# lucagiorgetti/Laplace-DQN-Snake-game

Measured on NVIDIA B200. Metric: snake_env_steps_per_sec, higher is better.
Workload: dtype u64 bitboards -> f32 obs

## Files before the change

laplace-dqn-snake-game_b200/csrc/snake_env.cu:

```cuda
#include <stdarg.h>
#include <string.h>

#include <new>
#include <mutex>
#include <type_traits>
#include <unordered_map>

#include <cuda.h>

#include "common.h"

#ifndef SNK_OBS_STORE_MODE
#define SNK_OBS_STORE_MODE 1
#endif
#if SNK_OBS_STORE_MODE == 1
#define SNK_OBS_STORE(p, v) (*(p) = (v))
#elif SNK_OBS_STORE_MODE == 2
#define SNK_OBS_STORE(p, v) __stwt((p), (v))
#else
#define SNK_OBS_STORE(p, v) __stcs((p), (v))
#endif

namespace snk {

static thread_local char g_err[512];
char *err_buf() { return g_err; }
int fail(int code, const char *fmt, ...) {
    va_list ap;
    va_start(ap, fmt);
    vsnprintf(g_err, sizeof(g_err), fmt, ap);
    va_end(ap);
    return code;
}

#ifndef SNK_TPB
#define SNK_TPB 256
#endif
#ifndef SNK_MINB
#define SNK_MINB 1
#endif
#ifndef SNK_UNROLL
#define SNK_UNROLL 4
#endif
constexpr int PHASE_B_UNROLL = SNK_UNROLL;
constexpr int TPB = SNK_TPB;
constexpr int MAX_FOOD = 64;
constexpr int PLANE_WORDS = 16;

constexpr int M_HR = 0, M_HC = 4, M_TR = 8, M_TC = 12, M_FR = 16, M_FC = 20, M_PFR = 24, M_PFC = 28;
constexpr int M_PD = 32, M_LEN = 34, M_T = 41, M_DONE = 51, M_ERR = 52;

constexpr u64 wall_bits(int lo_hi) {
    u64 lo = 0, hi = 0;
    for (int c = 0; c < 10; c++)
        for (int r = 0; r < 10; r++)
            if (r == 0 || r == 9 || c == 0 || c == 9) {
                int k = r + 10 * c;
                if (k < 64) lo |= 1ull << k; else hi |= 1ull << (k - 64);
            }
    return lo_hi ? hi : lo;
}
constexpr u64 WALL_LO = wall_bits(0), WALL_HI = wall_bits(1);

constexpr u64 INIT_OCC = (1ull << (6 + 0)) | (1ull << (7 + 0));
constexpr u64 INIT_MISC = (7ull << M_HR) | (1ull << M_HC) | (8ull << M_TR) | (1ull << M_TC) | (3ull << M_FR) |
                          (4ull << M_FC) | (3ull << M_PFR) | (4ull << M_PFC) | (0ull << M_PD) | (2ull << M_LEN);

struct FoodTable {
    uint8_t bit[MAX_FOOD];
    int n;
    __host__ __device__ u64 mask() const { return n >= 64 ? ~0ull : ((1ull << n) - 1ull); }
};

struct EnvState {
    u64 *occ, *pocc, *clo, *chi, *cons, *misc;
    float *ret;
};

__host__ __device__ constexpr int obs_bytes(int fmt) {
    switch (fmt) {
        case SNK_OBS_F32: return 800;
        case SNK_OBS_I8: return 200;
        case SNK_OBS_I64: return 1600;
        case SNK_OBS_PACKED2: return 50;
        case SNK_OBS_BITS: return 24;
        default: return 0;
    }
}

struct StepOutputs {
    float *reward;
    uint8_t *done;
    void *obs;
    uint8_t *mask;
    float *ep_return;
    int32_t *ep_score;
};

struct StepArgs {
    EnvState s;
    const uint8_t *act;
    const float *q;
    const float *u;
    const uint8_t *ridx;
    float eps;
    uint8_t *act_out;
    StepOutputs out;
    long long env_begin, env_end;
    u64 seed, step_counter;
    int auto_reset, is_abs;
    uint4 *sink;
    long long sink_base, sink_cap, sink_n;
    FoodTable food;
};

constexpr int REC_U4 = 8;

__host__ __device__ __forceinline__ u64 splitmix64(u64 x) {
    x += 0x9E3779B97F4A7C15ull;
    x = (x ^ (x >> 30)) * 0xBF58476D1CE4E5B9ull;
    x = (x ^ (x >> 27)) * 0x94D049BB133111EBull;
    return x ^ (x >> 31);
}

__device__ __forceinline__ void dir_delta(int d, int &dr, int &dc) {
    int s = (d & 1) ? 1 : -1;
    dr = (d & 2) ? 0 : s;
    dc = (d & 2) ? s : 0;
// ... 21 lines not shown
    if (b != b) return true;
    if (a < b) return true;
    if (a == b) return (__float_as_uint(a) >> 31) && !(__float_as_uint(b) >> 31);
    return false;
}
__device__ __forceinline__ int select_idx(float q0, float q1, float q2, float eps, float u, int ridx) {
    if (u < eps) return ridx;
    int best = 0;
    float qb = q0;
    if (jl_isless(qb, q1)) { best = 1; qb = q1; }
    if (jl_isless(qb, q2)) { best = 2; }
    return best;
}
__device__ __forceinline__ void internal_draw(u64 seed, u64 step, long long env, float &u, int &ridx) {
    u64 x = splitmix64(seed ^ splitmix64((u64)env * 0x100000001B3ull + step));
    u = (float)(x >> 40) * 5.9604644775390625e-08f;
    ridx = (int)((x & 0xFFFFFFull) % 3ull);
}

__device__ __forceinline__ void to_full(u64 occ, u64 &lo, u64 &hi) {
    u64 b0 = occ & 0xFF, b1 = (occ >> 8) & 0xFF, b2 = (occ >> 16) & 0xFF, b3 = (occ >> 24) & 0xFF;
    u64 b4 = (occ >> 32) & 0xFF, b5 = (occ >> 40) & 0xFF, b6 = (occ >> 48) & 0xFF, b7 = occ >> 56;
    lo = (b0 << 11) | (b1 << 21) | (b2 << 31) | (b3 << 41) | (b4 << 51) | (b5 << 61);
    hi = (b5 >> 3) | (b6 << 7) | (b7 << 17);
}
__device__ __forceinline__ void set_k(int r, int c, u64 &lo, u64 &hi) {
    int k = r + 10 * c;
    u64 b = 1ull << (k & 63);
    if (k < 64) lo |= b; else hi |= b;
}
__device__ __forceinline__ void board_bits(u64 occ, int fr, int fc, bool has_head, int hr, int hc, u64 &p0lo, u64 &p0hi,
                                           u64 &p1lo, u64 &p1hi) {
    u64 slo, shi;
    to_full(occ, slo, shi);
    if (has_head) set_k(hr, hc, slo, shi);
    u64 flo = WALL_LO, fhi = WALL_HI;
    if (fr != 0) set_k(fr, fc, flo, fhi);
    p0lo = slo | WALL_LO; p0hi = shi | WALL_HI;
    p1lo = flo & ~slo; p1hi = fhi & ~shi;
}
__device__ __forceinline__ u64 spread_nibbles(uint32_t x) {
    u64 v = x;
    v = (v | (v << 16)) & 0x0000FFFF0000FFFFull;
    v = (v | (v << 8)) & 0x00FF00FF00FF00FFull;
    v = (v | (v << 4)) & 0x0F0F0F0F0F0F0F0Full;
    return v;
}
__device__ __forceinline__ u64 unit_bytes(uint32_t p0, uint32_t p1) {
    const uint32_t ev = (p0 & 0x0F0F0F0Fu) | ((p1 << 4) & 0xF0F0F0F0u);
    const uint32_t od = ((p0 >> 4) & 0x0F0F0F0Fu) | (p1 & 0xF0F0F0F0u);
    return (u64)__byte_perm(ev, od, 0x5140) | ((u64)__byte_perm(ev, od, 0x7362) << 32);
}
template <bool PERM>
__device__ __forceinline__ u64 unit_word(uint32_t p0, uint32_t p1) {
    return PERM ? unit_bytes(p0, p1) : (spread_nibbles(p0) | (spread_nibbles(p1) << 4));
}
template <bool PERM = true>
__device__ __forceinline__ void board_planes(u64 occ, int fr, int fc, bool has_head, int hr, int hc, uint32_t *dst) {
    u64 p0lo, p0hi, p1lo, p1hi;
    board_bits(occ, fr, fc, has_head, hr, hc, p0lo, p0hi, p1lo, p1hi);
    u64 *d = reinterpret_cast<u64 *>(dst);
    d[0] = unit_word<PERM>((uint32_t)p0lo, (uint32_t)p1lo);
    d[1] = unit_word<PERM>((uint32_t)(p0lo >> 32), (uint32_t)(p1lo >> 32));
    d[2] = unit_word<PERM>((uint32_t)p0hi, (uint32_t)p1hi);
    d[3] = unit_word<PERM>((uint32_t)(p0hi >> 32), (uint32_t)(p1hi >> 32));
}
__device__ __forceinline__ void board_planes_reg(u64 occ, int fr, int fc, bool has_head, int hr, int hc, uint4 &a, uint4 &b) {
    u64 p0lo, p0hi, p1lo, p1hi;
    board_bits(occ, fr, fc, has_head, hr, hc, p0lo, p0hi, p1lo, p1hi);
    a = make_uint4((uint32_t)p0lo, (uint32_t)(p0lo >> 32), (uint32_t)p0hi, (uint32_t)(p0hi >> 32));
    b = make_uint4((uint32_t)p1lo, (uint32_t)(p1lo >> 32), (uint32_t)p1hi, (uint32_t)(p1hi >> 32));
}

__device__ __forceinline__ int cell_code(const uint32_t *pl, int k) {
    const uint32_t b = reinterpret_cast<const uint8_t *>(pl)[k >> 2];
    const int j = k & 3;
    return (int)(((b >> j) & 1u) | (((b >> (4 + j)) & 1u) << 1));
}
__device__ __forceinline__ int code_value(int code) { return code == 3 ? -1 : code; }

struct ObsTables {
    float4 f32[256];
};
template <int OBS>
__device__ __forceinline__ void fill_tables(ObsTables &tb, int tid, int nt = TPB) {
    if (OBS == SNK_OBS_F32 || OBS == SNK_OBS_I8 || OBS == SNK_OBS_PACKED2) {
        for (int i = tid; i < 256; i += nt) {
            int n0 = i & 15, n1 = i >> 4;
            float v[4];
            uint32_t bytes = 0, packed = 0;
            for (int j = 0; j < 4; j++) {
                int code = ((n0 >> j) & 1) | (((n1 >> j) & 1) << 1);
                v[j] = (float)code_value(code);
                bytes |= (uint32_t)(uint8_t)(int8_t)code_value(code) << (8 * j);
                packed |= (uint32_t)code << (2 * j);
            }
            if (OBS == SNK_OBS_F32) tb.f32[i] = make_float4(v[0], v[1], v[2], v[3]);
            else if (OBS == SNK_OBS_I8) reinterpret_cast<uint32_t *>(tb.f32)[i] = bytes;
            else reinterpret_cast<uint8_t *>(tb.f32)[i] = (uint8_t)packed;
        }
    }
}

template <bool STREAM, typename T>
__device__ __forceinline__ void obs_store(T *p, const T &v) {
    if (STREAM) __stcs(p, v); else SNK_OBS_STORE(p, v);
}
__device__ __forceinline__ uint32_t unit_index(const uint32_t *s_planes, int j) {
    const int e = (int)(((unsigned)j * 5243u) >> 18);
    const int qq = j - e * 50;
    const int f = qq >= 25;
    return reinterpret_cast<const uint8_t *>(s_planes)[e * (PLANE_WORDS * 4) + f * 32 + (qq - 25 * f)];
}
template <int OBS, int NT = TPB, int UNROLL = PHASE_B_UNROLL, bool STREAM = false>
__device__ __forceinline__ void expand_obs(void *obs, long long env0, int n_local, const uint32_t *s_planes,
                                           const ObsTables &tb, int tid) {
    if (OBS == SNK_OBS_F32) {
        const int total = n_local * 50;
        float4 *o32 = reinterpret_cast<float4 *>(obs) + env0 * 50;
#pragma unroll UNROLL
        for (int j = tid; j < total; j += NT) obs_store<STREAM>(o32 + j, tb.f32[unit_index(s_planes, j)]);
    } else if (OBS == SNK_OBS_I8) {
        constexpr int GP = NT / 25;
        uint8_t *base = reinterpret_cast<uint8_t *>(obs) + env0 * 200;
        const int n_pairs = (NT % 25 > 10) ? 0 : n_local >> 1;
        if ((reinterpret_cast<uintptr_t>(base) & 15u) == 0) {
            if (tid < GP * 25) {
                const int p0 = tid / 25, w = tid - 25 * p0;
                int off[4];
#pragma unroll
                for (int k = 0; k < 4; k++) {
                    const int uu = 4 * w + k, e2 = uu >= 50, qq = uu - 50 * e2;
                    off[k] = e2 * (PLANE_WORDS * 4) + (qq >= 25 ? 7 : 0) + qq;
                }
                const uint8_t *src = reinterpret_cast<const uint8_t *>(s_planes) + p0 * (2 * PLANE_WORDS * 4);
                const uint32_t *t32 = reinterpret_cast<const uint32_t *>(tb.f32);
                uint4 *o = reinterpret_cast<uint4 *>(base);
#pragma unroll 2
                for (int p = p0; p < n_pairs; p += GP, src += GP * (2 * PLANE_WORDS * 4))
                    obs_store<STREAM>(o + p * 25 + w, make_uint4(t32[src[off[0]]], t32[src[off[1]]], t32[src[off[2]]], t32[src[off[3]]]));
            }
        }
        const int done_units = (reinterpret_cast<uintptr_t>(base) & 15u) == 0 ? n_pairs * 100 : 0;
        for (int j = done_units + tid; j < n_local * 50; j += NT)
            reinterpret_cast<uint32_t *>(base)[j] = reinterpret_cast<const uint32_t *>(tb.f32)[unit_index(s_planes, j)];
    } else if (OBS == SNK_OBS_PACKED2) {
        uint8_t *base = reinterpret_cast<uint8_t *>(obs) + env0 * 50;
        const int total = n_local * 50;
        int done_units = 0;
        if ((reinterpret_cast<uintptr_t>(base) & 15u) == 0) {
            const int nvec = total / 16;
            uint4 *o = reinterpret_cast<uint4 *>(base);
#pragma unroll 2
            for (int v = tid; v < nvec; v += NT) {
                uint32_t w[4];
#pragma unroll
                for (int k = 0; k < 4; k++) {
                    uint32_t x = 0;
#pragma unroll
                    for (int b = 0; b < 4; b++)
                        x |= (uint32_t)reinterpret_cast<const uint8_t *>(tb.f32)[unit_index(s_planes, v * 16 + k * 4 + b)] << (8 * b);
                    w[k] = x;
                }
                obs_store<STREAM>(o + v, make_uint4(w[0], w[1], w[2], w[3]));
            }
            done_units = nvec * 16;
        }
        for (int j = done_units + tid; j < total; j += NT) base[j] = reinterpret_cast<const uint8_t *>(tb.f32)[unit_index(s_planes, j)];
    } else if (OBS == SNK_OBS_I64) {
        const int total = n_local * 100;
        longlong2 *o = reinterpret_cast<longlong2 *>(obs) + env0 * 100;
        for (int j = tid; j < total; j += NT) {
            int e = j / 100;
            int p = j - e * 100;
            int f = p >= 50;
            int k = 2 * (p - 50 * f);
            const uint32_t *pl = s_planes + e * PLANE_WORDS + f * 8;
            longlong2 v;
            v.x = code_value(cell_code(pl, k));
            v.y = code_value(cell_code(pl, k + 1));
            obs_store<STREAM>(o + j, v);
        }
    }
}

__device__ __forceinline__ uint32_t losing_mask3(u64 occ, u64 cons, int hr, int hc, int tr, int tc, int fr, int fc,
                                                 int pd, int t, u64 list_mask, const uint8_t *s_food_bit, int &err) {
    const bool cap = t >= 499;
    const u64 occ_nt = occ & ~(1ull << ((tr - 1) + 8 * (tc - 1)));
    uint32_t m = 0;
#pragma unroll
    for (int k = 0; k < 3; k++) {
        int d = av_dir(pd, k), dr, dc;
        dir_delta(d, dr, dc);
        int nr = hr + dr, nc = hc + dc;
        bool lose;
        if (nr == 0 || nr == 9 || nc == 0 || nc == 9) {
            lose = true;
        } else {
            int b = (nr - 1) + 8 * (nc - 1);
            if (fr != 0 && nr == fr && nc == fc) {
                lose = cap;
                if (food_search(occ | (1ull << b), cons, list_mask, s_food_bit) == -1) err |= SNK_ENV_ERR_FOOD;
            } else {
// ... 41 lines not shown
}
__device__ __forceinline__ void env_store(const Env &e, const EnvState &s, long long i, bool store_chi = true, bool store_cons = true) {
    const u64 misc = ((u64)e.hr << M_HR) | ((u64)e.hc << M_HC) | ((u64)e.tr << M_TR) | ((u64)e.tc << M_TC) |
                     ((u64)e.fr << M_FR) | ((u64)e.fc << M_FC) | ((u64)e.pfr << M_PFR) | ((u64)e.pfc << M_PFC) |
                     ((u64)e.pd << M_PD) | ((u64)e.len << M_LEN) | ((u64)e.t << M_T) | ((u64)e.dn << M_DONE) |
                     ((u64)e.err << M_ERR);
    s.occ[i] = e.occ; s.pocc[i] = e.pocc; s.clo[i] = e.clo; s.misc[i] = misc;
    if (store_chi) s.chi[i] = e.chi;
    if (store_cons) s.cons[i] = e.cons;
    s.ret[i] = e.ret;
}
__device__ __forceinline__ void env_reset(Env &e) {
    e.occ = INIT_OCC; e.pocc = INIT_OCC; e.clo = 0; e.chi = 0; e.cons = 0; e.ret = 0.0f;
    e.hr = 7; e.hc = 1; e.tr = 8; e.tc = 1; e.fr = 3; e.fc = 4; e.pfr = 3; e.pfc = 4; e.pd = 0; e.len = 2; e.t = 0; e.dn = 0;
}
template <bool WITH_MASK = true>
__device__ __forceinline__ float env_advance(Env &e, int &aidx, int is_abs, u64 list_mask, const uint8_t *s_food_bit,
                                             uint32_t &m3) {
    int d;
    if (is_abs) {
        d = aidx;
        if (d > 3) { e.err |= SNK_ENV_ERR_ACTION; d = 0; }
    } else {
        if (aidx > 2) { e.err |= SNK_ENV_ERR_ACTION; aidx = 0; }
        d = av_dir(e.pd, aidx);
    }
    int dr, dc;
    dir_delta(d, dr, dc);
    const int nr = e.hr + dr, nc = e.hc + dc;
    const bool wall = (nr == 0) | (nr == 9) | (nc == 0) | (nc == 9);
    const u64 nbit = wall ? 0ull : (1ull << ((nr - 1) + 8 * (nc - 1)));
    const bool eat = (e.fr != 0) & (nr == e.fr) & (nc == e.fc);
    const bool reverse = d == (e.pd ^ 1);
    e.pocc = e.occ; e.pfr = e.fr; e.pfc = e.fc;
    e.chi = (e.chi << 2) | (e.clo >> 62);
    e.clo = (e.clo << 2) | (u64)d;
    e.len++;
    bool self = false;
    float reward;
    if (eat) {
        reward = 1.0f;
        e.fr = 0; e.fc = 0;
        int i = food_search(e.occ | nbit, e.cons, list_mask, s_food_bit);
        if (i >= 0) {
            e.cons |= 1ull << i;
            int b = s_food_bit[i];
            e.fr = (b & 7) + 1; e.fc = (b >> 3) + 1;
        } else if (i == -1) {
            e.err |= SNK_ENV_ERR_FOOD;
        }
        e.occ |= nbit;
    } else {
        e.occ &= ~(1ull << ((e.tr - 1) + 8 * (e.tc - 1)));
        int c = chain_get(e.clo, e.chi, e.len - 2), er, ec;
        dir_delta(c, er, ec);
        e.tr += er; e.tc += ec;
        e.len--;
        reward = -0.01f;
        self = (e.occ & nbit) != 0ull;
        e.occ |= nbit;
    }
    e.t++;
    const bool lost = wall | self | reverse | (e.t >= 500);
    if (lost) reward = -1.0f;
    e.hr = nr; e.hc = nc; e.pd = d; e.dn = lost;
    e.ret += reward;
    m3 = 7u;
    if (WITH_MASK && !lost) m3 = losing_mask3(e.occ, e.cons, e.hr, e.hc, e.tr, e.tc, e.fr, e.fc, e.pd, e.t, list_mask, s_food_bit, e.err);
    return reward;
}

__device__ __forceinline__ void store_bits_record(void *obs, long long env, u64 pocc, int pfr, int pfc, u64 occ, int fr, int fc,
                                                  int hr, int hc, uint32_t m3, bool done, int aidx, float reward) {
    u64 *rec = reinterpret_cast<u64 *>(obs) + 3 * env;
    const uint32_t cells = (uint32_t)(pfr | (pfc << 4)) | ((uint32_t)(fr | (fc << 4)) << 8) | ((uint32_t)(hr | (hc << 4)) << 16) |
                           (((m3 & 7u) | ((uint32_t)done << 3) | (((uint32_t)aidx & 3u) << 4)) << 24);
    rec[0] = pocc;
    rec[1] = occ;
    rec[2] = (u64)cells | ((u64)__float_as_uint(reward) << 32);
}
__host__ __device__ constexpr bool obs_expands(int fmt) { return fmt != SNK_OBS_NONE && fmt != SNK_OBS_BITS; }

template <int OBS, bool SELECT, bool SINK>
__global__ void __launch_bounds__(TPB, (OBS == SNK_OBS_F32 || OBS == SNK_OBS_I64) ? SNK_MINB : 4) k_step(const __grid_constant__ StepArgs a) {
    __shared__ __align__(16) uint32_t s_planes[TPB * PLANE_WORDS];
    __shared__ ObsTables s_tb;
    __shared__ uint8_t s_food_bit[MAX_FOOD];

    const int tid = threadIdx.x;
    const long long env0 = a.env_begin + (long long)blockIdx.x * TPB;
    const long long rem = a.env_end - env0;
    const int n_local = rem < TPB ? (int)rem : TPB;
    const long long env = env0 + tid;

    if (tid < MAX_FOOD) s_food_bit[tid] = a.food.bit[tid];
    if (obs_expands(OBS)) fill_tables<OBS>(s_tb, tid);
    __syncthreads();

    if (tid < n_local) {
        Env e;
        env_load<SINK, true>(e, a.s, env);
        const bool chi_live = e.len >= CHI_FROM_LEN;
        const u64 cons_loaded = e.cons;
        const u64 list_mask = a.food.mask();
        const u64 occ_tm2 = e.pocc;
        const int fr_tm2 = e.pfr, fc_tm2 = e.pfc, pd_before = e.pd;

        int aidx;
        if (SELECT) {
            float q0 = a.q[3 * env], q1 = a.q[3 * env + 1], q2 = a.q[3 * env + 2];
            float u;
            int ri;
            if (a.u != nullptr && a.ridx != nullptr) {
                u = a.u[env];
                ri = a.ridx[env];
            } else {
                internal_draw(a.seed, a.step_counter, env, u, ri);
                if (a.u != nullptr) u = a.u[env];
                if (a.ridx != nullptr) ri = a.ridx[env];
            }
            aidx = select_idx(q0, q1, q2, a.eps, u, ri);
            if (a.act_out != nullptr) a.act_out[env] = (uint8_t)aidx;
        } else {
            aidx = a.act[env];
        }

        float reward = 0.0f;
        uint32_t m3 = 7u;
        if (!e.dn) reward = env_advance(e, aidx, a.is_abs, list_mask, s_food_bit, m3);

        if (a.out.reward != nullptr) a.out.reward[env] = reward;
        if (a.out.done != nullptr) a.out.done[env] = (uint8_t)e.dn;
        if (a.out.mask != nullptr) store_mask3(a.out.mask + 3 * env, m3);
        if (a.out.ep_return != nullptr) a.out.ep_return[env] = e.ret;
        if (a.out.ep_score != nullptr) a.out.ep_score[env] = e.len - 2;

        if (obs_expands(OBS)) {
            constexpr bool PERM = OBS != SNK_OBS_F32 && OBS != SNK_OBS_I64;
            board_planes<PERM>(e.pocc, e.pfr, e.pfc, false, 0, 0, s_planes + tid * PLANE_WORDS);
            board_planes<PERM>(e.occ, e.fr, e.fc, true, e.hr, e.hc, s_planes + tid * PLANE_WORDS + 8);
        }
        if (OBS == SNK_OBS_BITS)
            store_bits_record(a.out.obs, env, e.pocc, e.pfr, e.pfc, e.occ, e.fr, e.fc, e.hr, e.hc, m3, e.dn, aidx, reward);

        if (SINK) {
            const long long k = env - a.env_begin;
            if (k + a.sink_cap >= a.sink_n) {
                uint4 *rec = a.sink + ((a.sink_base + k) % a.sink_cap) * REC_U4;
                uint4 p0, p1;
                board_planes_reg(occ_tm2, fr_tm2, fc_tm2, false, 0, 0, p0, p1);
                rec[0] = p0; rec[1] = p1;
                board_planes_reg(e.pocc, e.pfr, e.pfc, false, 0, 0, p0, p1);
                rec[2] = p0; rec[3] = p1;
                board_planes_reg(e.occ, e.fr, e.fc, true, e.hr, e.hc, p0, p1);
                rec[4] = p0; rec[5] = p1;
                rec[6] = make_uint4(__float_as_uint(reward),
                                    (uint32_t)aidx | ((uint32_t)e.dn << 8) | (m3 << 16) | ((uint32_t)pd_before << 24),
                                    __float_as_uint(e.ret), (uint32_t)(e.len - 2));
                rec[7] = make_uint4((uint32_t)env, (uint32_t)e.t, 0u, 0u);
            }
        }

        if (e.dn && a.auto_reset) env_reset(e);
        env_store(e, a.s, env, chi_live || e.len >= CHI_FROM_LEN, e.cons != cons_loaded);
    }

    if (obs_expands(OBS)) {
        __syncthreads();
        expand_obs<OBS>(a.out.obs, env0, n_local, s_planes, s_tb, tid);
    }
}

struct RolloutArgs {
    EnvState s;
    const uint8_t *act;
    StepOutputs out;
    long long n;
    int steps, auto_reset, is_abs;
    long long *prof;
    FoodTable food;
};
#ifndef SNK_RTPB
#define SNK_RTPB 128
#endif
#ifndef SNK_WS_EPB
#define SNK_WS_EPB 16
#endif
constexpr int WS_EPB = SNK_WS_EPB;
constexpr int RTPB = SNK_RTPB;
template <int OBS, int EPB>
__global__ void __launch_bounds__(RTPB) k_rollout(const __grid_constant__ RolloutArgs a) {
    __shared__ __align__(16) uint32_t s_planes[EPB * PLANE_WORDS];
    __shared__ ObsTables s_tb;
    __shared__ uint8_t s_food_bit[MAX_FOOD];
    const int tid = threadIdx.x;
    const long long env0 = (long long)blockIdx.x * EPB;
    const long long rem = a.n - env0;
    const int n_local = rem < EPB ? (int)rem : EPB;
    const long long env = env0 + tid;
    const bool mine = tid < n_local;
    if (tid < MAX_FOOD) s_food_bit[tid] = a.food.bit[tid];
    if (OBS != SNK_OBS_NONE) fill_tables<OBS>(s_tb, tid, RTPB);
    __syncthreads();
    const u64 list_mask = a.food.mask();
    Env e;
    if (mine) env_load(e, a.s, env);
    const size_t obs_step = (size_t)a.n * obs_bytes(OBS);
    for (int t = 0; t < a.steps; t++) {
        if (mine) {
            const long long o = (long long)t * a.n + env;
            int aidx = a.act[o];
            float reward = 0.0f;
            uint32_t m3 = 7u;
            if (!e.dn) reward = env_advance(e, aidx, a.is_abs, list_mask, s_food_bit, m3);
            store_step_outputs(a.out, o, reward, e.dn, m3, e.ret, e.len - 2);
            if (OBS != SNK_OBS_NONE) {
                board_planes(e.pocc, e.pfr, e.pfc, false, 0, 0, s_planes + tid * PLANE_WORDS);
                board_planes(e.occ, e.fr, e.fc, true, e.hr, e.hc, s_planes + tid * PLANE_WORDS + 8);
            }
            if (e.dn && a.auto_reset) env_reset(e);
        }
        if (OBS != SNK_OBS_NONE) {
            __syncthreads();
            expand_obs<OBS, RTPB, 5, true>((uint8_t *)a.out.obs + (size_t)t * obs_step, env0, n_local, s_planes, s_tb, tid);
            __syncthreads();
        }
    }
    if (mine) env_store(e, a.s, env);
}

struct __align__(16) Handoff {
    u64 occ, pocc, cons;
    uint32_t pk;
    uint32_t pk2;
    float reward, ret;
    int score, pad;
};
__device__ __forceinline__ void nbar_sync(int id, int n) { asm volatile("bar.sync %0, %1;" ::"r"(id), "r"(n) : "memory"); }
__device__ __forceinline__ void nbar_arrive(int id, int n) { asm volatile("bar.arrive %0, %1;" ::"r"(id), "r"(n) : "memory"); }
#ifndef SNK_WS_XW
#define SNK_WS_XW 5
#endif
constexpr int WS_XW = SNK_WS_XW;
constexpr bool WS_STREAM = true;
constexpr int WS_THREADS = 32 * (3 + WS_XW);
constexpr int WS_BAR = 32 * (2 + WS_XW);

template <int OBS, int EPB>
__global__ void __launch_bounds__(WS_THREADS) k_rollout_ws(const __grid_constant__ RolloutArgs a) {
    static_assert(EPB <= 32, "one env per lane of the logic warp");
    constexpr int NX = 32 * WS_XW;
    constexpr bool TWO_MASK = OBS != SNK_OBS_F32 && OBS != SNK_OBS_I64;
// ... 64 lines not shown
            Handoff h;
            if (lane < n_local) h = s_hand[b][lane];
            __syncwarp();
            if (t + 2 < a.steps) nbar_arrive(EMPTY + b, WS_BAR);
            if (lane < n_local) {
                const int hr = (int)h.pk & 15, hc = (int)(h.pk >> 4) & 15, fr = (int)(h.pk >> 8) & 15, fc = (int)(h.pk >> 12) & 15;
                const int dn = (int)(h.pk >> 24) & 1;
                uint32_t m3 = 7u;
                if (!dn) {
                    int err = 0;
                    m3 = losing_mask3(h.occ, h.cons, hr, hc, (int)h.pk2 & 15, (int)(h.pk2 >> 4) & 15, fr, fc, (int)(h.pk2 >> 8) & 3,
                                      (int)(h.pk2 >> 10) & 1023, list_mask, s_food_bit, err);
                    if (err) atomicOr(&s_err[lane], err);
                }
                store_step_outputs(a.out, (long long)t * a.n + env0 + lane, h.reward, dn, m3, h.ret, h.score);
            }
            if (prof) p_role += clock64() - c0;
        }
        if (prof) { a.prof[2] = p_full; a.prof[3] = p_role; }
    } else if (warp < 2 + WS_XW) {
        const int et = tid - 64;
        const bool prof = a.prof != nullptr && blockIdx.x == 0 && et == 0;
        long long p_exp = 0, p_xfull = 0;
        const size_t obs_step = (size_t)a.n * obs_bytes(OBS);
        for (int t = 0; t < a.steps; t++) {
            const int b = t & 1;
            long long c0 = prof ? clock64() : 0;
            nbar_sync(FULL + b, WS_BAR);
            if (prof) { const long long c1 = clock64(); p_xfull += c1 - c0; c0 = c1; }
            const int j = et & 31, role = et >> 5;
            if (OBS != SNK_OBS_NONE && j < n_local && role < 2) {
                const Handoff h = s_hand[b][j];
                if (role == 0) {
                    board_planes(h.pocc, (int)(h.pk >> 16) & 15, (int)(h.pk >> 20) & 15, false, 0, 0, s_planes + j * PLANE_WORDS);
                } else {
                    board_planes(h.occ, (int)(h.pk >> 8) & 15, (int)(h.pk >> 12) & 15, true, (int)h.pk & 15, (int)(h.pk >> 4) & 15,
                                 s_planes + j * PLANE_WORDS + 8);
                }
            }
            if (t + 2 < a.steps) nbar_arrive(EMPTY + b, WS_BAR);
            if (OBS != SNK_OBS_NONE) {
                nbar_sync(XB, NX);
                expand_obs<OBS, NX, 5, WS_STREAM>((uint8_t *)a.out.obs + (size_t)t * obs_step, env0, n_local, s_planes, s_tb, et);
                nbar_sync(XB, NX);
                if (prof) p_exp += clock64() - c0;
            }
        }
        if (prof) { a.prof[4] = p_exp; a.prof[5] = p_xfull; }
    }
    __syncthreads();
    if (mine) {
        e.err |= s_err[lane];
        env_store(e, a.s, env);
    }
}

template <int OBS>
__global__ void __launch_bounds__(TPB) k_state(EnvState s, long long n, void *obs) {
    __shared__ __align__(16) uint32_t s_planes[TPB * PLANE_WORDS];
    __shared__ ObsTables s_tb;
    const int tid = threadIdx.x;
    const long long env0 = (long long)blockIdx.x * TPB;
    const int n_local = (n - env0) < TPB ? (int)(n - env0) : TPB;
    if (OBS == SNK_OBS_BITS) {
        if (tid < n_local) {
            const long long env = env0 + tid;
            const u64 misc = s.misc[env];
            store_bits_record(obs, env, s.pocc[env], (int)(misc >> M_PFR) & 15, (int)(misc >> M_PFC) & 15, s.occ[env],
                              (int)(misc >> M_FR) & 15, (int)(misc >> M_FC) & 15, (int)(misc >> M_HR) & 15, (int)(misc >> M_HC) & 15,
                              0u, ((misc >> M_DONE) & 1ull) != 0, 0, 0.0f);
        }
        return;
    }
    fill_tables<OBS>(s_tb, tid);
    if (tid < n_local) {
        long long env = env0 + tid;
        u64 misc = s.misc[env];
        board_planes(s.pocc[env], (int)(misc >> M_PFR) & 15, (int)(misc >> M_PFC) & 15, false, 0, 0,
                     s_planes + tid * PLANE_WORDS);
        board_planes(s.occ[env], (int)(misc >> M_FR) & 15, (int)(misc >> M_FC) & 15, true, (int)(misc >> M_HR) & 15,
                     (int)(misc >> M_HC) & 15, s_planes + tid * PLANE_WORDS + 8);
    }
    __syncthreads();
    expand_obs<OBS>(obs, env0, n_local, s_planes, s_tb, tid);
}

template <int OBS>
__global__ void __launch_bounds__(TPB) k_patch_reset(long long n, const uint8_t *__restrict__ done, void *obs) {
    __shared__ __align__(16) uint32_t s_pl[8];
    __shared__ ObsTables s_tb;
    __shared__ int s_list[TPB];
    __shared__ int s_cnt;
    const int tid = threadIdx.x;
    const long long env0 = (long long)blockIdx.x * TPB;
    if (OBS == SNK_OBS_BITS) {
        if (env0 + tid < n && done[env0 + tid] != 0) {
            u64 *rec = reinterpret_cast<u64 *>(obs) + 3 * (env0 + tid);
            rec[0] = INIT_OCC;
            rec[1] = INIT_OCC;
            rec[2] = (rec[2] & ~0xFFFFFFull) | (u64)((3 | (4 << 4)) | ((3 | (4 << 4)) << 8) | ((7 | (1 << 4)) << 16));
        }
        return;
    }
    fill_tables<OBS>(s_tb, tid);
    if (tid == 0) {
        s_cnt = 0;
        board_planes(INIT_OCC, 3, 4, false, 0, 0, s_pl);
    }
    __syncthreads();
    if (env0 + tid < n && done[env0 + tid] != 0) s_list[atomicAdd(&s_cnt, 1)] = tid;
    __syncthreads();
    const int cnt = s_cnt;
    if (OBS == SNK_OBS_I64) {
        for (int j = tid; j < cnt * 100; j += TPB) {
            const int e = j / 100, p = j - e * 100, k = 2 * (p % 50);
            longlong2 v;
            v.x = code_value(cell_code(s_pl, k));
            v.y = code_value(cell_code(s_pl, k + 1));
            reinterpret_cast<longlong2 *>(obs)[(env0 + s_list[e]) * 100 + p] = v;
        }
    } else {
        for (int j = tid; j < cnt * 50; j += TPB) {
            const int e = j / 50, qq = j - e * 50;
            const uint32_t idx = reinterpret_cast<const uint8_t *>(s_pl)[qq % 25];
            const long long o = (env0 + s_list[e]) * 50 + qq;
            if (OBS == SNK_OBS_F32) reinterpret_cast<float4 *>(obs)[o] = s_tb.f32[idx];
            else if (OBS == SNK_OBS_I8) reinterpret_cast<uint32_t *>(obs)[o] = reinterpret_cast<const uint32_t *>(s_tb.f32)[idx];
            else reinterpret_cast<uint8_t *>(obs)[o] = reinterpret_cast<const uint8_t *>(s_tb.f32)[idx];
        }
    }
}

__global__ void k_reset(EnvState s, long long n) {
    long long i = (long long)blockIdx.x * blockDim.x + threadIdx.x;
    if (i >= n) return;
    s.occ[i] = INIT_OCC; s.pocc[i] = INIT_OCC; s.clo[i] = 0; s.chi[i] = 0; s.cons[i] = 0;
    s.misc[i] = INIT_MISC; s.ret[i] = 0.0f;
}

__global__ void k_available_actions(EnvState s, long long n, uint8_t *out) {
    long long i = (long long)blockIdx.x * blockDim.x + threadIdx.x;
    if (i >= n) return;
    int pd = (int)(s.misc[i] >> M_PD) & 3;
    for (int k = 0; k < 3; k++) out[3 * i + k] = (uint8_t)av_dir(pd, k);
}

__global__ void k_losing_mask(EnvState s, long long n, uint8_t *out, FoodTable food) {
    __shared__ uint8_t s_food_bit[MAX_FOOD];
    if (threadIdx.x < MAX_FOOD) s_food_bit[threadIdx.x] = food.bit[threadIdx.x];
    __syncthreads();
    long long i = (long long)blockIdx.x * blockDim.x + threadIdx.x;
    if (i >= n) return;
    u64 misc = s.misc[i];
    uint32_t m3 = 7u;
    if (!((misc >> M_DONE) & 1ull)) {
        int err = (int)(misc >> M_ERR) & 15, err0 = err;
        m3 = losing_mask3(s.occ[i], s.cons[i], (int)(misc >> M_HR) & 15, (int)(misc >> M_HC) & 15,
                          (int)(misc >> M_TR) & 15, (int)(misc >> M_TC) & 15, (int)(misc >> M_FR) & 15,
                          (int)(misc >> M_FC) & 15, (int)(misc >> M_PD) & 3, (int)(misc >> M_T) & 1023, food.mask(),
                          s_food_bit, err);
        if (err != err0) s.misc[i] = (misc & ~(15ull << M_ERR)) | ((u64)err << M_ERR);
    }
    store_mask3(out + 3 * i, m3);
}

__global__ void k_select(long long n, const float *q, float eps, const float *u, const uint8_t *ridx, u64 seed,
                         u64 step, uint8_t *out) {
// ... 379 lines not shown
    k_reset<<<nblocks(h->n, 256), 256, 0, h->stream>>>(h->s, h->n);
    SNK_CUDA(cudaGetLastError());
    *out = h;
    return SNK_OK;
}

int snk_destroy(snk_handle h) {
    if (h == nullptr) return SNK_OK;
    DeviceGuard guard(h->device);
    if (h->own_stream) cudaStreamSynchronize(h->own_stream);
    for (int i = 0; i < 2; i++) if (h->copy_stream[i]) cudaStreamSynchronize(h->copy_stream[i]);
    void *ptrs[] = {h->s.occ, h->s.pocc, h->s.clo, h->s.chi, h->s.cons, h->s.misc, h->s.ret, h->d_count, h->d_q, h->d_u,
                    h->d_reward, h->d_ep_return, h->d_ridx, h->d_act, h->d_done, h->d_mask, h->d_ep_score, h->d_obs};
    for (void *p : ptrs) if (p) cudaFree(p);
    for (int i = 0; i < 2; i++) if (h->copy_stream[i]) cudaStreamDestroy(h->copy_stream[i]);
    if (h->ev_in) cudaEventDestroy(h->ev_in);
    if (h->ev_done) cudaEventDestroy(h->ev_done);
    for (int i = 0; i < 64; i++) if (h->ev_chunk[i]) cudaEventDestroy(h->ev_chunk[i]);
    for (int i = 0; i < 64; i++) if (h->ev_up[i]) cudaEventDestroy(h->ev_up[i]);
    if (h->own_stream) cudaStreamDestroy(h->own_stream);
    delete h;
    return SNK_OK;
}

int snk_reset(snk_handle h) {
    SNK_CHECK_HANDLE(h);
    k_reset<<<nblocks(h->n, 256), 256, 0, h->stream>>>(h->s, h->n);
    SNK_CUDA(cudaGetLastError());
    return SNK_OK;
}

int snk_set_food_list_host(snk_handle h, const uint8_t *cells_rc_host, int n) {
    SNK_CHECK_HANDLE(h);
    SNK_REQUIRE(cells_rc_host != nullptr || n == 0, "null list");
    FoodTable ft;
    int rc = set_food(ft, cells_rc_host, n);
    if (rc != SNK_OK) return rc;
    SNK_CUDA(cudaStreamSynchronize(h->stream));
    h->food = ft;
    return SNK_OK;
}

int snk_set_stream(snk_handle h, void *cuda_stream) {
    SNK_CHECK_HANDLE(h);
    SNK_CUDA(cudaStreamSynchronize(h->stream));
    h->stream = (cudaStream_t)cuda_stream;
    return SNK_OK;
}
int snk_use_own_stream(snk_handle h) {
    SNK_CHECK_HANDLE(h);
    SNK_CUDA(cudaStreamSynchronize(h->stream));
    h->stream = h->own_stream;
    return SNK_OK;
}
int snk_get_stream(snk_handle h, void **cuda_stream) {
    SNK_CHECK_HANDLE(h);
    SNK_REQUIRE(cuda_stream != nullptr, "null out");
    *cuda_stream = (void *)h->stream;
    return SNK_OK;
}
int snk_set_seed(snk_handle h, uint64_t seed) {
    SNK_CHECK_HANDLE(h);
    h->seed = seed; h->step_counter = 0;
    return SNK_OK;
}
int snk_sync(snk_handle h) {
    SNK_CHECK_HANDLE(h);
    SNK_CUDA(cudaStreamSynchronize(h->stream));
    SNK_CUDA(cudaStreamSynchronize(h->copy_stream[0]));
    return SNK_OK;
}
int64_t snk_num_envs(snk_handle h) { return h ? h->n : 0; }

int snk_available_actions(snk_handle h, uint8_t *dirs_3xN) {
    SNK_CHECK_HANDLE(h);
    SNK_REQUIRE(dirs_3xN != nullptr, "null out");
    k_available_actions<<<nblocks(h->n, 256), 256, 0, h->stream>>>(h->s, h->n, dirs_3xN);
    SNK_CUDA(cudaGetLastError());
    return SNK_OK;
}

static int launch_step(StepArgs &a, int obs_fmt, bool select, long long begin, long long end, cudaStream_t st) {
    a.env_begin = begin; a.env_end = end;
    unsigned grid = nblocks(end - begin, TPB);
    if (grid == 0) return SNK_OK;
    return launch_obs_fmt<SNK_OBS_NONE, SNK_OBS_F32, SNK_OBS_I8, SNK_OBS_I64, SNK_OBS_PACKED2, SNK_OBS_BITS>(obs_fmt, [&](auto fmt) {
        constexpr int FMT = decltype(fmt)::value;
        if (a.sink != nullptr) {
            if (select) k_step<FMT, true, true><<<grid, TPB, 0, st>>>(a);
            else k_step<FMT, false, true><<<grid, TPB, 0, st>>>(a);
        } else {
            if (select) k_step<FMT, true, false><<<grid, TPB, 0, st>>>(a);
            else k_step<FMT, false, false><<<grid, TPB, 0, st>>>(a);
        }
    });
}

static StepArgs step_args(snk_handle h, const float *q, float eps, const float *u, const uint8_t *ridx, uint8_t *act_idx,
                          const StepOutputs &out, const snk_replay_s *r) {
    StepArgs a;
    memset(&a, 0, sizeof(a));
    a.s = h->s; a.food = h->food; a.seed = h->seed; a.step_counter = h->step_counter;
    a.auto_reset = (h->flags & SNK_AUTO_RESET) ? 1 : 0;
    a.q = q; a.eps = eps; a.u = u; a.ridx = ridx;
    if (q != nullptr) a.act_out = act_idx; else a.act = act_idx;
    a.out = out;
    if (r != nullptr) { a.sink = r->ring; a.sink_base = r->total; a.sink_cap = r->capacity; a.sink_n = h->n; }
    return a;
}

static int step_plain(snk_handle h, const uint8_t *act, int is_abs, float *reward, uint8_t *done) {
    StepArgs a = step_args(h, nullptr, 0.0f, nullptr, nullptr, nullptr, {reward, done}, nullptr);
    a.act = act; a.is_abs = is_abs;
    int rc = launch_step(a, SNK_OBS_NONE, false, 0, h->n, h->stream);
    h->step_counter++;
    return rc;
}

int snk_step(snk_handle h, const uint8_t *act_idx, float *reward, uint8_t *done) {
    SNK_CHECK_HANDLE(h);
    SNK_REQUIRE(act_idx != nullptr, "null actions");
    return step_plain(h, act_idx, 0, reward, done);
}

int snk_step_abs(snk_handle h, const uint8_t *dir, float *reward, uint8_t *done) {
    SNK_CHECK_HANDLE(h);
    SNK_REQUIRE(dir != nullptr, "null directions");
    return step_plain(h, dir, 1, reward, done);
}

static int check_step_inputs(const char *fn, const float *q, const uint8_t *act_idx, const void *obs, int obs_fmt) {
    if (q == nullptr && act_idx == nullptr) return fail(SNK_ERR_INVALID, "%s: need q (select) or act_idx (input)", fn);
    if (obs_fmt != SNK_OBS_NONE && obs == nullptr) return fail(SNK_ERR_INVALID, "%s: obs_fmt given without an obs buffer", fn);
    return SNK_OK;
}
static int check_replay(const char *fn, snk_handle h, const snk_replay_s *r, const char *what) {
    if (r->device != h->device) return fail(SNK_ERR_INVALID, "%s: replay ring and env live on different devices", fn);
    if (!(h->flags & SNK_AUTO_RESET))
        return fail(SNK_ERR_UNSUPPORTED, "%s needs an env created with SNK_AUTO_RESET (every env must step)", what);
    return SNK_OK;
}

static int step_fused_impl(const char *fn, snk_handle h, snk_replay_s *r, const float *q, float eps, const float *u,
                           const uint8_t *ridx, uint8_t *act_idx, float *reward, uint8_t *done, void *obs, int obs_fmt,
                           uint8_t *mask, float *ep_return, int32_t *ep_score) {
    if (h == nullptr) return fail(SNK_ERR_INVALID, "%s: null handle", fn);
    DeviceGuard guard(h->device);
    int rc = r != nullptr ? check_replay(fn, h, r, fn) : SNK_OK;
    if (rc == SNK_OK) rc = check_step_inputs(fn, q, act_idx, obs, obs_fmt);
    if (rc != SNK_OK) return rc;
    if (obs_fmt != SNK_OBS_NONE && ((uintptr_t)obs & 15u) != 0) return fail(SNK_ERR_INVALID, "%s: obs must be 16-byte aligned", fn);
    StepArgs a = step_args(h, q, eps, u, ridx, act_idx, {reward, done, obs, mask, ep_return, ep_score}, r);
    rc = launch_step(a, obs ? obs_fmt : SNK_OBS_NONE, q != nullptr, 0, h->n, h->stream);
    h->step_counter++;
    if (rc == SNK_OK && r != nullptr) r->total += h->n;
    return rc;
}

int snk_step_fused(snk_handle h, const float *q, float eps, const float *u, const uint8_t *ridx, uint8_t *act_idx,
                   float *reward, uint8_t *done, void *obs, int obs_fmt, uint8_t *mask, float *ep_return,
                   int32_t *ep_score) {
    return step_fused_impl(__func__, h, nullptr, q, eps, u, ridx, act_idx, reward, done, obs, obs_fmt, mask, ep_return, ep_score);
}

int snk_rollout_fused(snk_handle h, const uint8_t *act_TxN, int64_t T, int is_abs, float *reward, uint8_t *done, void *obs,
                      int obs_fmt, uint8_t *mask, float *ep_return, int32_t *ep_score) {
    SNK_CHECK_HANDLE(h);
    SNK_REQUIRE(act_TxN != nullptr && T > 0 && T <= (1 << 20), "bad argument");
    SNK_REQUIRE(obs_fmt == SNK_OBS_NONE || obs != nullptr, "obs_fmt given without an obs buffer");
    SNK_REQUIRE(obs == nullptr || ((uintptr_t)obs & 15u) == 0, "obs must be 16-byte aligned");
    RolloutArgs a;
    memset(&a, 0, sizeof(a));
    a.s = h->s; a.food = h->food; a.act = act_TxN; a.out = {reward, done, obs, mask, ep_return, ep_score};
    a.n = h->n; a.steps = (int)T; a.is_abs = is_abs;
    a.prof = g_rollout_prof;
    a.auto_reset = (h->flags & SNK_AUTO_RESET) ? 1 : 0;
// ... 190 lines not shown
    cudaFree(r->d_bad);
    if (r->stage) cudaFree(r->stage);
    delete r;
    return SNK_OK;
}
int snk_replay_clear(snk_replay r) {
    SNK_REQUIRE(r != nullptr, "null replay");
    r->total = 0;
    return SNK_OK;
}
int snk_replay_length(snk_replay r, int64_t *length, int64_t *position) {
    SNK_REQUIRE(r != nullptr, "null replay");
    if (length) *length = r->total < r->capacity ? r->total : r->capacity;
    if (position) *position = r->total < r->capacity ? 1 : ((r->total - r->capacity) % r->capacity) + 1;
    return SNK_OK;
}

int snk_step_fused_store(snk_handle h, snk_replay r, const float *q, float eps, const float *u, const uint8_t *ridx,
                         uint8_t *act_idx, float *reward, uint8_t *done, void *obs, int obs_fmt, uint8_t *mask,
                         float *ep_return, int32_t *ep_score) {
    SNK_REQUIRE(r != nullptr, "null replay");
    return step_fused_impl(__func__, h, r, q, eps, u, ridx, act_idx, reward, done, obs, obs_fmt, mask, ep_return, ep_score);
}

int snk_replay_gather(snk_replay r, const int64_t *idx, int64_t B, float *states, float *next_states, uint8_t *actions,
                      float *rewards, uint8_t *dones, uint8_t *mask, float *ep_return, int32_t *score, void *cuda_stream) {
    SNK_REQUIRE(r != nullptr && idx != nullptr && B >= 0, "bad argument");
    SNK_REQUIRE((((uintptr_t)states | (uintptr_t)next_states) & 15u) == 0, "state buffers must be 16-byte aligned");
    if (B == 0) return SNK_OK;
    DeviceGuard guard(r->device);
    k_replay_gather<<<nblocks(B, GATHER_S), 128, 0, (cudaStream_t)cuda_stream>>>(
        r->ring, r->capacity, (const long long *)idx, B, states, next_states, actions, rewards, dones, mask, ep_return,
        score, r->d_bad);
    SNK_CUDA(cudaGetLastError());
    return SNK_OK;
}

int snk_replay_sample_indices(snk_replay r, uint64_t seed, int64_t B, int64_t *idx_out, void *cuda_stream) {
    SNK_REQUIRE(r != nullptr && idx_out != nullptr, "bad argument");
    const long long n = r->total < r->capacity ? r->total : r->capacity;
    SNK_REQUIRE(B >= 0 && B <= n, "cannot sample more distinct transitions than the buffer holds");
    if (B == 0) return SNK_OK;
    DeviceGuard guard(r->device);
    const u64 key = splitmix64(seed ^ splitmix64(r->draws++));
    k_replay_sample<<<nblocks(B, 256), 256, 0, (cudaStream_t)cuda_stream>>>(n, B, key, (long long *)idx_out);
    SNK_CUDA(cudaGetLastError());
    return SNK_OK;
}

int snk_replay_bad_index_host(snk_replay r, int *flag) {
    SNK_REQUIRE(r != nullptr && flag != nullptr, "bad argument");
    DeviceGuard guard(r->device);
    SNK_CUDA(cudaMemcpy(flag, r->d_bad, sizeof(int), cudaMemcpyDeviceToHost));
    return SNK_OK;
}

static int step_fused_host_impl(snk_handle h, snk_replay_s *r, const float *q, float eps, const float *u, const uint8_t *ridx,
                                uint8_t *act_idx, float *reward, uint8_t *done, void *obs, int obs_fmt, uint8_t *mask,
                                float *ep_return, int32_t *ep_score) {
    SNK_CHECK_HANDLE(h);
    int rc = check_step_inputs(__func__, q, act_idx, obs, obs_fmt);
    if (rc == SNK_OK && r != nullptr) rc = check_replay(__func__, h, r, "storing transitions");
    if (rc != SNK_OK) return rc;
    const size_t n = (size_t)h->n;
    const size_t opb = obs ? obs_bytes(obs_fmt) : 0;
    if (obs && opb == 0) return fail(SNK_ERR_INVALID, "unknown obs_fmt %d", obs_fmt);
    SNK_CUDA(ensure(&h->d_act, n));
    if (q) { SNK_CUDA(ensure(&h->d_q, 12 * n)); }
    if (u) { SNK_CUDA(ensure(&h->d_u, 4 * n)); }
    if (ridx) { SNK_CUDA(ensure(&h->d_ridx, n)); }
    if (reward) { SNK_CUDA(ensure(&h->d_reward, 4 * n)); }
    if (done) { SNK_CUDA(ensure(&h->d_done, n)); }
    if (mask) { SNK_CUDA(ensure(&h->d_mask, 3 * n)); }
    if (ep_return) { SNK_CUDA(ensure(&h->d_ep_return, 4 * n)); }
    if (ep_score) { SNK_CUDA(ensure(&h->d_ep_score, 4 * n)); }
    if (opb && (rc = ensure_obs_staging(h, opb * n)) != SNK_OK) return rc;
    if ((rc = staging_guard(h)) != SNK_OK) return rc;
    cudaStream_t st = h->stream, down = h->copy_stream[0], up = h->copy_stream[1];
    StepArgs a = step_args(h, q ? h->d_q : nullptr, eps, u ? h->d_u : nullptr, ridx ? h->d_ridx : nullptr, act_idx ? h->d_act : nullptr,
                           {reward ? h->d_reward : nullptr, done ? h->d_done : nullptr, opb ? h->d_obs : nullptr,
                            mask ? h->d_mask : nullptr, ep_return ? h->d_ep_return : nullptr, ep_score ? h->d_ep_score : nullptr},
                           r);
    const long long align = TPB * 8;
    const size_t traffic = (opb + 26) * n;
    int n_chunks = (int)((traffic + (SNK_HOST_CHUNK_MB << 20) - 1) / (SNK_HOST_CHUNK_MB << 20));
    if (n_chunks < 1) n_chunks = 1;
    if (n_chunks > 16) n_chunks = 16;
    const long long per = ((h->n + n_chunks - 1) / n_chunks + align - 1) / align * align;
    SNK_CUDA(cudaEventRecord(h->ev_in, st));
    SNK_CUDA(cudaStreamWaitEvent(up, h->ev_in, 0));
    int ci = 0;
    for (long long b = 0; b < h->n; b += per, ci++) {
        const long long e = b + per < h->n ? b + per : h->n;
        const size_t nb = (size_t)(e - b);
        if (q) SNK_CUDA(cudaMemcpyAsync(h->d_q + 3 * b, q + 3 * b, 12 * nb, cudaMemcpyHostToDevice, up));
        if (u) SNK_CUDA(cudaMemcpyAsync(h->d_u + b, u + b, 4 * nb, cudaMemcpyHostToDevice, up));
        if (ridx) SNK_CUDA(cudaMemcpyAsync(h->d_ridx + b, ridx + b, nb, cudaMemcpyHostToDevice, up));
        if (!q) SNK_CUDA(cudaMemcpyAsync(h->d_act + b, act_idx + b, nb, cudaMemcpyHostToDevice, up));
        SNK_CUDA(cudaEventRecord(h->ev_up[ci], up));
        SNK_CUDA(cudaStreamWaitEvent(st, h->ev_up[ci], 0));
        if ((rc = launch_step(a, opb ? obs_fmt : SNK_OBS_NONE, q != nullptr, b, e, st)) != SNK_OK) return rc;
        SNK_CUDA(cudaEventRecord(h->ev_chunk[ci], st));
        SNK_CUDA(cudaStreamWaitEvent(down, h->ev_chunk[ci], 0));
        if (opb) SNK_CUDA(cudaMemcpyAsync((char *)obs + opb * b, (char *)h->d_obs + opb * b, opb * nb, cudaMemcpyDeviceToHost, down));
    }
    if (mask) SNK_CUDA(cudaMemcpyAsync(mask, h->d_mask, 3 * n, cudaMemcpyDeviceToHost, down));
    if (reward) SNK_CUDA(cudaMemcpyAsync(reward, h->d_reward, 4 * n, cudaMemcpyDeviceToHost, down));
    if (done) SNK_CUDA(cudaMemcpyAsync(done, h->d_done, n, cudaMemcpyDeviceToHost, down));
    if (ep_return) SNK_CUDA(cudaMemcpyAsync(ep_return, h->d_ep_return, 4 * n, cudaMemcpyDeviceToHost, down));
    if (ep_score) SNK_CUDA(cudaMemcpyAsync(ep_score, h->d_ep_score, 4 * n, cudaMemcpyDeviceToHost, down));
    if (q && act_idx) SNK_CUDA(cudaMemcpyAsync(act_idx, h->d_act, n, cudaMemcpyDeviceToHost, down));
    h->step_counter++;
    if (r != nullptr) r->total += h->n;
    SNK_CUDA(cudaEventRecord(h->ev_done, down));
    return SNK_OK;
}

int snk_step_fused_host(snk_handle h, const float *q, float eps, const float *u, const uint8_t *ridx, uint8_t *act_idx,
                        float *reward, uint8_t *done, void *obs, int obs_fmt, uint8_t *mask, float *ep_return,
                        int32_t *ep_score) {
    return step_fused_host_impl(h, nullptr, q, eps, u, ridx, act_idx, reward, done, obs, obs_fmt, mask, ep_return, ep_score);
}

int snk_step_fused_store_host(snk_handle h, snk_replay r, const float *q, float eps, const float *u, const uint8_t *ridx,
                              uint8_t *act_idx, float *reward, uint8_t *done, void *obs, int obs_fmt, uint8_t *mask,
                              float *ep_return, int32_t *ep_score) {
    SNK_REQUIRE(r != nullptr, "null replay");
    return step_fused_host_impl(h, r, q, eps, u, ridx, act_idx, reward, done, obs, obs_fmt, mask, ep_return, ep_score);
}

int snk_state_host(snk_handle h, void *obs_host, int obs_fmt) {
    SNK_CHECK_HANDLE(h);
    SNK_REQUIRE(obs_host != nullptr, "null out");
    const size_t opb = obs_bytes(obs_fmt);
    if (opb == 0) return fail(SNK_ERR_INVALID, "unknown obs_fmt %d", obs_fmt);
    return get_host(h, obs_host, opb * (size_t)h->n, [&](void *d) { return snk_state(h, d, obs_fmt); });
}

int snk_losing_mask_host(snk_handle h, uint8_t *mask_3xN_host) {
    SNK_CHECK_HANDLE(h);
    SNK_REQUIRE(mask_3xN_host != nullptr, "null out");
    return get_host(h, mask_3xN_host, 3 * (size_t)h->n, [&](void *d) { return snk_losing_mask(h, (uint8_t *)d); });
}

int snk_available_actions_host(snk_handle h, uint8_t *dirs_3xN_host) {
    SNK_CHECK_HANDLE(h);
    SNK_REQUIRE(dirs_3xN_host != nullptr, "null out");
    return get_host(h, dirs_3xN_host, 3 * (size_t)h->n, [&](void *d) { return snk_available_actions(h, (uint8_t *)d); });
}

static int scalars_host(snk_handle h, int which, void *out_host, size_t elem) {
    SNK_CHECK_HANDLE(h);
    SNK_REQUIRE(out_host != nullptr, "null out");
    return get_host(h, out_host, elem * (size_t)h->n, [&](void *d) { return scalars(h, which, d); });
}
int snk_get_score_host(snk_handle h, int32_t *score_host) { return scalars_host(h, 0, score_host, 4); }
int snk_get_done_host(snk_handle h, uint8_t *done_host) { return scalars_host(h, 1, done_host, 1); }
int snk_get_error_flags_host(snk_handle h, uint8_t *flags_host) { return scalars_host(h, 2, flags_host, 1); }
int snk_get_steps_host(snk_handle h, int32_t *steps_host) { return scalars_host(h, 3, steps_host, 4); }

int snk_replay_gather_host(snk_replay r, const int64_t *idx_host, int64_t B, float *states, float *next_states, uint8_t *actions,
                           float *rewards, uint8_t *dones, uint8_t *mask, void *cuda_stream) {
    SNK_REQUIRE(r != nullptr && idx_host != nullptr && B >= 0, "bad argument");
    if (B == 0) return SNK_OK;
    DeviceGuard guard(r->device);
    cudaStream_t st = (cudaStream_t)cuda_stream;
// ... 27 lines not shown
```

Baseline: 8.790 billion.

## Compute f32 obs words arithmetically and shrink F32 step CTA to 128 threads

For the f32 observation path, the step kernel no longer builds or reads a shared-memory float4 lookup table. Each output float4 is now computed from the cell byte with bit tricks and byte_perm. The F32 step kernel also gets its own block size of 128 threads, with launch bounds and grid computed per format, and the default unroll goes from 4 to 8. The aim is to cut table-fill work, shared-memory bank traffic and per-CTA shared footprint, at the cost of a few extra ALU ops per stored unit.

Measured after the change: 9.066 billion, median of 6. 3.1% higher.

```diff
diff --git a/laplace-dqn-snake-game_b200/csrc/snake_env.cu b/laplace-dqn-snake-game_b200/csrc/snake_env.cu
--- a/laplace-dqn-snake-game_b200/csrc/snake_env.cu
+++ b/laplace-dqn-snake-game_b200/csrc/snake_env.cu
@@ -40,10 +40,17 @@
 #define SNK_MINB 1
 #endif
 #ifndef SNK_UNROLL
-#define SNK_UNROLL 4
+#define SNK_UNROLL 8
 #endif
 constexpr int PHASE_B_UNROLL = SNK_UNROLL;
 constexpr int TPB = SNK_TPB;
+#ifndef SNK_F32_TPB
+#define SNK_F32_TPB 128
+#endif
+#ifndef SNK_F32_MINB
+#define SNK_F32_MINB 1
+#endif
+__host__ __device__ constexpr int step_tpb(int obs) { return obs == SNK_OBS_F32 ? SNK_F32_TPB : TPB; }
 constexpr int MAX_FOOD = 64;
 constexpr int PLANE_WORDS = 16;
 
@@ -231,9 +238,9 @@
 struct ObsTables {
     float4 f32[256];
 };
-template <int OBS>
+template <int OBS, bool F32_TABLE = true>
 __device__ __forceinline__ void fill_tables(ObsTables &tb, int tid, int nt = TPB) {
-    if (OBS == SNK_OBS_F32 || OBS == SNK_OBS_I8 || OBS == SNK_OBS_PACKED2) {
+    if ((OBS == SNK_OBS_F32 && F32_TABLE) || OBS == SNK_OBS_I8 || OBS == SNK_OBS_PACKED2) {
         for (int i = tid; i < 256; i += nt) {
             int n0 = i & 15, n1 = i >> 4;
             float v[4];
@@ -261,14 +268,27 @@
     const int f = qq >= 25;
     return reinterpret_cast<const uint8_t *>(s_planes)[e * (PLANE_WORDS * 4) + f * 32 + (qq - 25 * f)];
 }
-template <int OBS, int NT = TPB, int UNROLL = PHASE_B_UNROLL, bool STREAM = false>
+__device__ __forceinline__ uint4 f32_unit_words(uint32_t b) {
+    uint32_t t = (b & 0x0Fu) | ((b & 0xF0u) << 12);
+    t = (t | (t << 6)) & 0x03030303u;
+    t = (t | (t << 3)) & 0x11111111u;
+    const uint32_t sel = (t | (t >> 15)) & 0xFFFFu;
+    const uint32_t top = __byte_perm(0xBF403F00u, 0u, sel);
+    return make_uint4(__byte_perm(top, 0u, 0x0444) | ((b << 23) & 0x00800000u), __byte_perm(top, 0u, 0x1444) | ((b << 22) & 0x00800000u),
+                      __byte_perm(top, 0u, 0x2444) | ((b << 21) & 0x00800000u), __byte_perm(top, 0u, 0x3444) | ((b << 20) & 0x00800000u));
+}
+template <int OBS, int NT = TPB, int UNROLL = PHASE_B_UNROLL, bool STREAM = false, bool F32_WORDS = false>
 __device__ __forceinline__ void expand_obs(void *obs, long long env0, int n_local, const uint32_t *s_planes,
                                            const ObsTables &tb, int tid) {
     if (OBS == SNK_OBS_F32) {
         const int total = n_local * 50;
         float4 *o32 = reinterpret_cast<float4 *>(obs) + env0 * 50;
 #pragma unroll UNROLL
-        for (int j = tid; j < total; j += NT) obs_store<STREAM>(o32 + j, tb.f32[unit_index(s_planes, j)]);
+        for (int j = tid; j < total; j += NT) {
+            const uint32_t b = unit_index(s_planes, j);
+            if (F32_WORDS) obs_store<STREAM>(reinterpret_cast<uint4 *>(o32) + j, f32_unit_words(b));
+            else obs_store<STREAM>(o32 + j, tb.f32[b]);
+        }
     } else if (OBS == SNK_OBS_I8) {
         constexpr int GP = NT / 25;
         uint8_t *base = reinterpret_cast<uint8_t *>(obs) + env0 * 200;
@@ -476,19 +496,20 @@
 __host__ __device__ constexpr bool obs_expands(int fmt) { return fmt != SNK_OBS_NONE && fmt != SNK_OBS_BITS; }
 
 template <int OBS, bool SELECT, bool SINK>
-__global__ void __launch_bounds__(TPB, (OBS == SNK_OBS_F32 || OBS == SNK_OBS_I64) ? SNK_MINB : 4) k_step(const __grid_constant__ StepArgs a) {
-    __shared__ __align__(16) uint32_t s_planes[TPB * PLANE_WORDS];
+__global__ void __launch_bounds__(step_tpb(OBS), OBS == SNK_OBS_F32 ? SNK_F32_MINB : OBS == SNK_OBS_I64 ? SNK_MINB : 4) k_step(const __grid_constant__ StepArgs a) {
+    constexpr int NT = step_tpb(OBS);
+    __shared__ __align__(16) uint32_t s_planes[NT * PLANE_WORDS];
     __shared__ ObsTables s_tb;
     __shared__ uint8_t s_food_bit[MAX_FOOD];
 
     const int tid = threadIdx.x;
-    const long long env0 = a.env_begin + (long long)blockIdx.x * TPB;
+    const long long env0 = a.env_begin + (long long)blockIdx.x * NT;
     const long long rem = a.env_end - env0;
-    const int n_local = rem < TPB ? (int)rem : TPB;
+    const int n_local = rem < NT ? (int)rem : NT;
     const long long env = env0 + tid;
 
     if (tid < MAX_FOOD) s_food_bit[tid] = a.food.bit[tid];
-    if (obs_expands(OBS)) fill_tables<OBS>(s_tb, tid);
+    if (obs_expands(OBS)) fill_tables<OBS, false>(s_tb, tid, NT);
     __syncthreads();
 
     if (tid < n_local) {
@@ -561,7 +582,7 @@
 
     if (obs_expands(OBS)) {
         __syncthreads();
-        expand_obs<OBS>(a.out.obs, env0, n_local, s_planes, s_tb, tid);
+        expand_obs<OBS, NT, PHASE_B_UNROLL, false, true>(a.out.obs, env0, n_local, s_planes, s_tb, tid);
     }
 }
 
@@ -792,7 +813,7 @@
                      (int)(misc >> M_HC) & 15, s_planes + tid * PLANE_WORDS + 8);
     }
     __syncthreads();
-    expand_obs<OBS>(obs, env0, n_local, s_planes, s_tb, tid);
+    expand_obs<OBS, TPB, 4>(obs, env0, n_local, s_planes, s_tb, tid);
 }
 
 template <int OBS>
@@ -1338,16 +1359,16 @@
 
 static int launch_step(StepArgs &a, int obs_fmt, bool select, long long begin, long long end, cudaStream_t st) {
     a.env_begin = begin; a.env_end = end;
-    unsigned grid = nblocks(end - begin, TPB);
-    if (grid == 0) return SNK_OK;
+    if (end <= begin) return SNK_OK;
     return launch_obs_fmt<SNK_OBS_NONE, SNK_OBS_F32, SNK_OBS_I8, SNK_OBS_I64, SNK_OBS_PACKED2, SNK_OBS_BITS>(obs_fmt, [&](auto fmt) {
-        constexpr int FMT = decltype(fmt)::value;
+        constexpr int FMT = decltype(fmt)::value, NT = step_tpb(FMT);
+        const unsigned grid = nblocks(end - begin, NT);
         if (a.sink != nullptr) {
-            if (select) k_step<FMT, true, true><<<grid, TPB, 0, st>>>(a);
-            else k_step<FMT, false, true><<<grid, TPB, 0, st>>>(a);
+            if (select) k_step<FMT, true, true><<<grid, NT, 0, st>>>(a);
+            else k_step<FMT, false, true><<<grid, NT, 0, st>>>(a);
         } else {
-            if (select) k_step<FMT, true, false><<<grid, TPB, 0, st>>>(a);
-            else k_step<FMT, false, false><<<grid, TPB, 0, st>>>(a);
+            if (select) k_step<FMT, true, false><<<grid, NT, 0, st>>>(a);
+            else k_step<FMT, false, false><<<grid, NT, 0, st>>>(a);
         }
     });
 }
@@ -1704,6 +1725,7 @@
                             mask ? h->d_mask : nullptr, ep_return ? h->d_ep_return : nullptr, ep_score ? h->d_ep_score : nullptr},
                            r);
     const long long align = TPB * 8;
+    static_assert(TPB * 8 % SNK_F32_TPB == 0, "chunks start on a CTA boundary of every format");
     const size_t traffic = (opb + 26) * n;
     int n_chunks = (int)((traffic + (SNK_HOST_CHUNK_MB << 20) - 1) / (SNK_HOST_CHUNK_MB << 20));
     if (n_chunks < 1) n_chunks = 1;
```
